# lajoiepy/cslam

Hardware: AMD Instinct MI355X
Metric: keyframes/sec (extract+match) on 100kx4096-D bank (higher is better)
Workload: dtype f32

## Files before the change

cslam_amd/csrc/wino_chain.hip:

```cpp
#include "common.h"
#include "pairs.h"
#include <hip/hip_fp16.h>

typedef float cf4 __attribute__((ext_vector_type(4)));
typedef unsigned cu2 __attribute__((ext_vector_type(2)));
typedef unsigned cu4 __attribute__((ext_vector_type(4)));

__device__ __forceinline__ void wc_at4(const cf4 m0, const cf4 m1, const cf4 m2, const cf4 m3, const cf4 m4, const cf4 m5,
                                       cf4 &s0, cf4 &s1, cf4 &s2, cf4 &s3) {
    const cf4 a = m1 + m2, bq = m1 - m2, c = m3 + m4, e = m3 - m4;
    s0 = m0 + a + c;
    s1 = bq + 2.0f * e;
    s2 = a + 4.0f * c;
    s3 = bq + 8.0f * e + m5;
}
__device__ __forceinline__ void wc_bt4(cf4 &d0, cf4 &d1, cf4 &d2, cf4 &d3, cf4 &d4, cf4 &d5) {
    const cf4 r0 = 4.0f * d0 - 5.0f * d2 + d4;
    const cf4 r1 = -4.0f * (d1 + d2) + d3 + d4;
    const cf4 r2 = 4.0f * (d1 - d2) - d3 + d4;
    const cf4 r3 = 2.0f * (d3 - d1) - d2 + d4;
    const cf4 r4 = 2.0f * (d1 - d3) - d2 + d4;
    const cf4 r5 = 4.0f * d1 - 5.0f * d3 + d5;
    d0 = r0; d1 = r1; d2 = r2; d3 = r3; d4 = r4; d5 = r5;
}

#define WC_THREADS 128
#define WC_RING 9

struct WcArgs {
    const float *mb;
    __half *vb;
    unsigned moff, voff;
    float *rp;
    int64_t mplane, vplane, mrow, vrow;
    int H, TH, Wr, tj;
    float inv, sc;
    cf4 bv;
    cf4 clim;
    bool odd;
};

template <int CG, bool OUT, bool LOAD, bool IN>
__device__ __forceinline__ void wc_step(const WcArgs &a, const int r, cf4 (&m)[36], float &vmax) {
    if (OUT) {
        cf4 s[4][6];
#pragma unroll
        for (int j = 0; j < 6; ++j)
            wc_at4(m[j], m[6 + j], m[12 + j], m[18 + j], m[24 + j], m[30 + j], s[0][j], s[1][j], s[2][j], s[3][j]);
#pragma unroll
        for (int i = 0; i < 4; ++i) {
            cf4 o[4];
            wc_at4(s[i][0], s[i][1], s[i][2], s[i][3], s[i][4], s[i][5], o[0], o[1], o[2], o[3]);
            const int h = 4 * r + i;
            float *row = a.rp + ((h % WC_RING) * a.Wr + 4 * a.tj) * CG;
            const cf4 lim = h < a.H ? a.clim : (cf4)(0.0f);
#pragma unroll
            for (int j = 0; j < 4; ++j) {
                cf4 v = __builtin_elementwise_max(o[j] * a.inv + a.bv, (cf4)(0.0f));
                v = __builtin_elementwise_min(v, (cf4)(lim[j]));
                vmax = fmaxf(fmaxf(vmax, fmaxf(v.x, v.y)), fmaxf(v.z, v.w));
                *(cf4 *)(row + j * CG) = v;
            }
        }
    }
    __syncthreads();
    if (LOAD) {
        const float *p = a.mb + (r + 1) * a.mrow;
#pragma unroll
        for (int q = 0; q < 36; ++q) m[q] = __builtin_nontemporal_load((const cf4 *)(p + q * a.mplane + a.moff));
    }
    if (IN) {
        const int h0 = 4 * (r - 1) - 1, w0 = 4 * a.tj - 1;
        const int Hr = 4 * a.TH;
        cf4 d[6][6];
#pragma unroll
        for (int i = 0; i < 6; ++i) {
            const int hh = h0 + i;
            const float *row = a.rp + ((hh + WC_RING) % WC_RING) * a.Wr * CG;
#pragma unroll
            for (int j = 0; j < 6; ++j) {
                const int ww = w0 + j;
                const bool in = (hh >= 0) & (hh < Hr) & (ww >= 0) & (ww < a.Wr);
                cf4 v = *(const cf4 *)(row + (j == 0 ? max(ww, 0) : j == 5 ? min(ww, a.Wr - 1) : ww) * CG);
                asm("" : "+v"(v));
                d[i][j] = in ? v * a.sc : (cf4)(0.0f);
            }
        }
#pragma unroll
        for (int j = 0; j < 6; ++j) wc_bt4(d[0][j], d[1][j], d[2][j], d[3][j], d[4][j], d[5][j]);
#pragma unroll
        for (int i = 0; i < 6; ++i) wc_bt4(d[i][0], d[i][1], d[i][2], d[i][3], d[i][4], d[i][5]);
        __half *o = a.vb + (r - 1) * a.vrow;
#pragma unroll
        for (int i = 0; i < 6; ++i)
#pragma unroll
            for (int j = 0; j < 6; ++j) {
                const cf4 v = d[i][j];
                const __half2 h0v = __floats2half2_rn(v.x, v.y), h1v = __floats2half2_rn(v.z, v.w);
                const __half2 l0v = __floats2half2_rn(sub_half<0>(v.x, h0v), sub_half<1>(v.y, h0v));
                const __half2 l1v = __floats2half2_rn(sub_half<0>(v.z, h1v), sub_half<1>(v.w, h1v));
                cu2 hi, lo;
                hi.x = *(const unsigned *)&h0v; hi.y = *(const unsigned *)&h1v;
                lo.x = *(const unsigned *)&l0v; lo.y = *(const unsigned *)&l1v;
                const cu2 give = a.odd ? hi : lo;
                cu2 got;
                got.x = (unsigned)__builtin_amdgcn_mov_dpp((int)give.x, 0xB1, 0xF, 0xF, true);
                got.y = (unsigned)__builtin_amdgcn_mov_dpp((int)give.y, 0xB1, 0xF, 0xF, true);
                cu4 v16;
                if (a.odd) { v16.x = got.x; v16.y = got.y; v16.z = lo.x; v16.w = lo.y; }
                else { v16.x = hi.x; v16.y = hi.y; v16.z = got.x; v16.w = got.y; }
                __builtin_nontemporal_store(v16, (cu4 *)(o + (6 * i + j) * a.vplane + a.voff));
            }
    }
    __syncthreads();
}

template <int CG>
__global__ __launch_bounds__(WC_THREADS) void wino4_chain_h2_kernel(const float *__restrict__ M, const float *__restrict__ bias,
                                                                     int B, int H, int W, int C,
                                                                     const unsigned *__restrict__ vscale, float inv_su,
                                                                     const unsigned *__restrict__ amax_x, float wl1, float bmax,
                                                                     unsigned *__restrict__ amax_out,
                                                                     unsigned *__restrict__ bound_out, __half *__restrict__ V2) {
    extern __shared__ __attribute__((aligned(16))) float ring[];
    __shared__ unsigned wg_amax;
    constexpr int C4G = CG / 4;
    WcArgs a;
    a.H = H;
    a.TH = (H + 3) >> 2;
    const int TW = (W + 3) >> 2;
    a.Wr = 4 * TW;
    const int ncg = C / CG;
    const int b = blockIdx.x / ncg, cg = blockIdx.x - b * ncg;
    a.tj = threadIdx.x / C4G;
    const int c4 = threadIdx.x % C4G;
    const int c = cg * CG + 4 * c4;
    const int64_t T = (int64_t)B * a.TH * TW;
    const int64_t t0 = (int64_t)b * a.TH * TW;
    if (threadIdx.x == 0) wg_amax = 0u;

    a.inv = inv_su / scale_le_327_68(__uint_as_float(*vscale));
    const float bound = fmaf(__uint_as_float(*amax_x), wl1, bmax);
    a.sc = scale_le_327_68(bound);
    if (blockIdx.x == 0 && threadIdx.x == 0) *bound_out = __float_as_uint(bound);
    a.bv = bias ? *(const cf4 *)(bias + c) : (cf4)(0.0f);
#pragma unroll
    for (int j = 0; j < 4; ++j) a.clim[j] = 4 * a.tj + j < W ? __builtin_inff() : 0.0f;
    a.odd = threadIdx.x & 1;
    a.mplane = T * C;
    a.vplane = T * 2 * C;
    a.mrow = (int64_t)TW * C;
    a.vrow = (int64_t)TW * 2 * C;
    a.mb = M + t0 * C + cg * CG;
    a.vb = V2 + t0 * 2 * C + cg * 2 * CG;
    a.moff = a.tj * C + 4 * c4;
    a.voff = a.tj * 2 * C + (c4 >> 3) * 64 + (4 * c4 & 31) + (a.odd ? 32 - 4 : 0);
    a.rp = ring + 4 * c4;
    float vmax = 0.0f;

    cf4 m[36];
#pragma unroll
    for (int q = 0; q < 36; ++q) m[q] = __builtin_nontemporal_load((const cf4 *)(a.mb + q * a.mplane + a.moff));
    const int TH = a.TH;
    if (TH == 1) {
        wc_step<CG, true, false, false>(a, 0, m, vmax);
    } else {
        wc_step<CG, true, true, false>(a, 0, m, vmax);
#pragma unroll 1
        for (int r = 1; r < TH - 1; ++r) wc_step<CG, true, true, true>(a, r, m, vmax);
        wc_step<CG, true, false, true>(a, TH - 1, m, vmax);
    }
    wc_step<CG, false, false, true>(a, TH, m, vmax);
#pragma unroll
    for (int o = 32; o > 0; o >>= 1) vmax = fmaxf(vmax, __shfl_xor(vmax, o, 64));
    if ((threadIdx.x & 63) == 0) atomicMax(&wg_amax, __float_as_uint(vmax));
    __syncthreads();
    if (threadIdx.x == 0 && wg_amax > *(volatile unsigned *)amax_out) atomicMax(amax_out, wg_amax);
}

template <int CG>
static int wino4_chain_launch(const float *d_M, const float *d_bias, int B, int H, int W, int C, const unsigned *d_vscale,
                              float inv_su, const unsigned *d_amax_x, float wl1, float bmax, unsigned *d_amax_out,
                              unsigned *d_bound_out, void *d_V2, void *stream) {
    const size_t lds = (size_t)WC_RING * 4 * ((W + 3) / 4) * CG * sizeof(float);
    ARG_CHECK(lds <= 144 * 1024, "map too wide for the LDS ring");
    static DeviceOnce once;
    int dev;
    if (once.todo(&dev)) {
        HIP_TRY(hipFuncSetAttribute((const void *)wino4_chain_h2_kernel<CG>, hipFuncAttributeMaxDynamicSharedMemorySize, 144 * 1024));
        once.done(dev);
    }
    hipLaunchKernelGGL(wino4_chain_h2_kernel<CG>, dim3((unsigned)((int64_t)B * (C / CG))), dim3(((W + 3) / 4) * (CG / 4)), lds, (hipStream_t)stream,
                       d_M, d_bias, B, H, W, C, d_vscale, inv_su, d_amax_x, wl1, bmax, d_amax_out, d_bound_out, (__half *)d_V2);
    HIP_TRY(hipGetLastError());
    return CSLAM_OK;
}

CSLAM_API int cslam_wino4_chain_h2_dev(const float *d_M, const float *d_bias, int B, int H, int W, int C,
                                       const unsigned *d_vscale, float inv_su, const unsigned *d_amax_x, float wl1, float bmax,
                                       unsigned *d_amax_out, unsigned *d_bound_out, void *d_V2, void *stream) {
    PTR_DEVICE(d_M);
    ARG_CHECK(d_M && d_V2 && d_vscale && d_amax_x && d_amax_out && d_bound_out, "NULL argument");
    ARG_CHECK(B >= 1 && H >= 1 && W >= 1, "empty map");
    ARG_CHECK(C >= 32 && (C % 32) == 0, "C must be a multiple of 32");
    ARG_CHECK(inv_su > 0.0f && wl1 >= 0.0f && bmax >= 0.0f, "inv_su must be positive, wl1 and bmax non-negative");
    const int TW = (W + 3) / 4;
    ARG_CHECK(TW <= 16, "maps wider than 64 pixels stay on the separate transforms");
    ARG_CHECK((int64_t)B * (C / 32) < (1LL << 31), "too many frames for one launch");
    if (TW <= 4 && (C % 128) == 0)
        return wino4_chain_launch<128>(d_M, d_bias, B, H, W, C, d_vscale, inv_su, d_amax_x, wl1, bmax, d_amax_out, d_bound_out, d_V2, stream);
    if (TW <= 8 && (C % 64) == 0)
        return wino4_chain_launch<64>(d_M, d_bias, B, H, W, C, d_vscale, inv_su, d_amax_x, wl1, bmax, d_amax_out, d_bound_out, d_V2, stream);
    return wino4_chain_launch<32>(d_M, d_bias, B, H, W, C, d_vscale, inv_su, d_amax_x, wl1, bmax, d_amax_out, d_bound_out, d_V2, stream);
}
```

Before: 19040.

## Pad LDS ring with zero halo and prescale on write to drop bounds checks

The LDS ring now has a one-pixel zero-padded border per row (Wp = 4*TW+1) and is zero-initialised, so the input-transform reads no longer need per-element bounds tests, clamping, or multiplication by the scale. The scale factor moves to the output-transform write side, and the final empty step writes zeros instead of skipping the write. The B^T transform is rewritten with explicit FMAs under contract(off) to keep rounding deterministic. Ablation variants selected by an env var are added, but only when built with CSLAM_ABLATIONS; the cost is a little more LDS and an initial zero-fill.

```diff
diff --git a/cslam_amd/csrc/wino_chain.hip b/cslam_amd/csrc/wino_chain.hip
--- a/cslam_amd/csrc/wino_chain.hip
+++ b/cslam_amd/csrc/wino_chain.hip
@@ -14,13 +14,22 @@
     s2 = a + 4.0f * c;
     s3 = bq + 8.0f * e + m5;
 }
+template <bool FUSED>
+__device__ __forceinline__ cf4 wc_4a5b(const cf4 a, const cf4 b) {
+#pragma clang fp contract(off)
+    if (FUSED) return __builtin_elementwise_fma((cf4)(-5.0f), b, 4.0f * a);
+    const cf4 t = 5.0f * b;
+    return __builtin_elementwise_fma((cf4)(4.0f), a, -t);
+}
+template <bool DOWN>
 __device__ __forceinline__ void wc_bt4(cf4 &d0, cf4 &d1, cf4 &d2, cf4 &d3, cf4 &d4, cf4 &d5) {
-    const cf4 r0 = 4.0f * d0 - 5.0f * d2 + d4;
-    const cf4 r1 = -4.0f * (d1 + d2) + d3 + d4;
-    const cf4 r2 = 4.0f * (d1 - d2) - d3 + d4;
-    const cf4 r3 = 2.0f * (d3 - d1) - d2 + d4;
-    const cf4 r4 = 2.0f * (d1 - d3) - d2 + d4;
-    const cf4 r5 = 4.0f * d1 - 5.0f * d3 + d5;
+#pragma clang fp contract(off)
+    const cf4 r0 = wc_4a5b<DOWN>(d0, d2) + d4;
+    const cf4 r1 = __builtin_elementwise_fma((cf4)(-4.0f), d1 + d2, d3) + d4;
+    const cf4 r2 = __builtin_elementwise_fma((cf4)(4.0f), d1 - d2, -d3) + d4;
+    const cf4 r3 = __builtin_elementwise_fma((cf4)(2.0f), d3 - d1, -d2) + d4;
+    const cf4 r4 = __builtin_elementwise_fma((cf4)(2.0f), d1 - d3, -d2) + d4;
+    const cf4 r5 = wc_4a5b<false>(d1, d3) + d5;
     d0 = r0; d1 = r1; d2 = r2; d3 = r3; d4 = r4; d5 = r5;
 }
 
@@ -33,35 +42,42 @@
     unsigned moff, voff;
     float *rp;
     int64_t mplane, vplane, mrow, vrow;
-    int H, TH, Wr, tj;
+    int H, Wp;
     float inv, sc;
     cf4 bv;
     cf4 clim;
     bool odd;
 };
 
-template <int CG, bool OUT, bool LOAD, bool IN>
-__device__ __forceinline__ void wc_step(const WcArgs &a, const int r, cf4 (&m)[36], float &vmax) {
+template <int CG, bool OUT, bool LOAD, bool IN, int DBG>
+__device__ __forceinline__ void wc_step(const WcArgs &a, const int r, cf4 (&m)[36], float &vmax, unsigned &sink) {
     if (OUT) {
         cf4 s[4][6];
 #pragma unroll
-        for (int j = 0; j < 6; ++j)
-            wc_at4(m[j], m[6 + j], m[12 + j], m[18 + j], m[24 + j], m[30 + j], s[0][j], s[1][j], s[2][j], s[3][j]);
+        for (int j = 0; j < 6; ++j) {
+            if (DBG == 3) s[0][j] = s[1][j] = s[2][j] = s[3][j] = m[j] + m[6 + j] + m[12 + j] + m[18 + j] + m[24 + j] + m[30 + j];
+            else wc_at4(m[j], m[6 + j], m[12 + j], m[18 + j], m[24 + j], m[30 + j], s[0][j], s[1][j], s[2][j], s[3][j]);
+        }
 #pragma unroll
         for (int i = 0; i < 4; ++i) {
             cf4 o[4];
-            wc_at4(s[i][0], s[i][1], s[i][2], s[i][3], s[i][4], s[i][5], o[0], o[1], o[2], o[3]);
+            if (DBG == 3) { o[0] = s[i][0] + s[i][4]; o[1] = s[i][1] + s[i][5]; o[2] = s[i][2]; o[3] = s[i][3]; }
+            else wc_at4(s[i][0], s[i][1], s[i][2], s[i][3], s[i][4], s[i][5], o[0], o[1], o[2], o[3]);
             const int h = 4 * r + i;
-            float *row = a.rp + ((h % WC_RING) * a.Wr + 4 * a.tj) * CG;
+            float *row = a.rp + ((h % WC_RING) * a.Wp + 1) * CG;
             const cf4 lim = h < a.H ? a.clim : (cf4)(0.0f);
 #pragma unroll
             for (int j = 0; j < 4; ++j) {
                 cf4 v = __builtin_elementwise_max(o[j] * a.inv + a.bv, (cf4)(0.0f));
                 v = __builtin_elementwise_min(v, (cf4)(lim[j]));
                 vmax = fmaxf(fmaxf(vmax, fmaxf(v.x, v.y)), fmaxf(v.z, v.w));
-                *(cf4 *)(row + j * CG) = v;
+                *(cf4 *)(row + j * CG) = v * a.sc;
             }
         }
+    } else {
+        float *row = a.rp + (((4 * r) % WC_RING) * a.Wp + 1) * CG;
+#pragma unroll
+        for (int j = 0; j < 4; ++j) *(cf4 *)(row + j * CG) = (cf4)(0.0f);
     }
     __syncthreads();
     if (LOAD) {
@@ -69,27 +85,19 @@
 #pragma unroll
         for (int q = 0; q < 36; ++q) m[q] = __builtin_nontemporal_load((const cf4 *)(p + q * a.mplane + a.moff));
     }
-    if (IN) {
-        const int h0 = 4 * (r - 1) - 1, w0 = 4 * a.tj - 1;
-        const int Hr = 4 * a.TH;
+    if (IN && DBG != 2) {
+        const int h0 = 4 * (r - 1) - 1;
         cf4 d[6][6];
 #pragma unroll
         for (int i = 0; i < 6; ++i) {
-            const int hh = h0 + i;
-            const float *row = a.rp + ((hh + WC_RING) % WC_RING) * a.Wr * CG;
-#pragma unroll
-            for (int j = 0; j < 6; ++j) {
-                const int ww = w0 + j;
-                const bool in = (hh >= 0) & (hh < Hr) & (ww >= 0) & (ww < a.Wr);
-                cf4 v = *(const cf4 *)(row + (j == 0 ? max(ww, 0) : j == 5 ? min(ww, a.Wr - 1) : ww) * CG);
-                asm("" : "+v"(v));
-                d[i][j] = in ? v * a.sc : (cf4)(0.0f);
-            }
+            const float *row = a.rp + ((h0 + i + WC_RING) % WC_RING) * a.Wp * CG;
+#pragma unroll
+            for (int j = 0; j < 6; ++j) d[i][j] = *(const cf4 *)(row + j * CG);
         }
 #pragma unroll
-        for (int j = 0; j < 6; ++j) wc_bt4(d[0][j], d[1][j], d[2][j], d[3][j], d[4][j], d[5][j]);
-#pragma unroll
-        for (int i = 0; i < 6; ++i) wc_bt4(d[i][0], d[i][1], d[i][2], d[i][3], d[i][4], d[i][5]);
+        for (int j = 0; j < 6; ++j) wc_bt4<true>(d[0][j], d[1][j], d[2][j], d[3][j], d[4][j], d[5][j]);
+#pragma unroll
+        for (int i = 0; i < 6; ++i) wc_bt4<false>(d[i][0], d[i][1], d[i][2], d[i][3], d[i][4], d[i][5]);
         __half *o = a.vb + (r - 1) * a.vrow;
 #pragma unroll
         for (int i = 0; i < 6; ++i)
@@ -109,13 +117,14 @@
                 cu4 v16;
                 if (a.odd) { v16.x = got.x; v16.y = got.y; v16.z = lo.x; v16.w = lo.y; }
                 else { v16.x = hi.x; v16.y = hi.y; v16.z = got.x; v16.w = got.y; }
-                __builtin_nontemporal_store(v16, (cu4 *)(o + (6 * i + j) * a.vplane + a.voff));
+                if (DBG == 1) sink ^= v16.x ^ v16.y ^ v16.z ^ v16.w;
+                else __builtin_nontemporal_store(v16, (cu4 *)(o + (6 * i + j) * a.vplane + a.voff));
             }
     }
     __syncthreads();
 }
 
-template <int CG>
+template <int CG, int DBG>
 __global__ __launch_bounds__(WC_THREADS) void wino4_chain_h2_kernel(const float *__restrict__ M, const float *__restrict__ bias,
                                                                      int B, int H, int W, int C,
                                                                      const unsigned *__restrict__ vscale, float inv_su,
@@ -127,16 +136,15 @@
     constexpr int C4G = CG / 4;
     WcArgs a;
     a.H = H;
-    a.TH = (H + 3) >> 2;
-    const int TW = (W + 3) >> 2;
-    a.Wr = 4 * TW;
+    const int TH = (H + 3) >> 2, TW = (W + 3) >> 2;
+    a.Wp = 4 * TW + 1;
     const int ncg = C / CG;
     const int b = blockIdx.x / ncg, cg = blockIdx.x - b * ncg;
-    a.tj = threadIdx.x / C4G;
+    const int tj = threadIdx.x / C4G;
     const int c4 = threadIdx.x % C4G;
     const int c = cg * CG + 4 * c4;
-    const int64_t T = (int64_t)B * a.TH * TW;
-    const int64_t t0 = (int64_t)b * a.TH * TW;
+    const int64_t T = (int64_t)B * TH * TW;
+    const int64_t t0 = (int64_t)b * TH * TW;
     if (threadIdx.x == 0) wg_amax = 0u;
 
     a.inv = inv_su / scale_le_327_68(__uint_as_float(*vscale));
@@ -145,7 +153,7 @@
     if (blockIdx.x == 0 && threadIdx.x == 0) *bound_out = __float_as_uint(bound);
     a.bv = bias ? *(const cf4 *)(bias + c) : (cf4)(0.0f);
 #pragma unroll
-    for (int j = 0; j < 4; ++j) a.clim[j] = 4 * a.tj + j < W ? __builtin_inff() : 0.0f;
+    for (int j = 0; j < 4; ++j) a.clim[j] = 4 * tj + j < W ? __builtin_inff() : 0.0f;
     a.odd = threadIdx.x & 1;
     a.mplane = T * C;
     a.vplane = T * 2 * C;
@@ -153,24 +161,32 @@
     a.vrow = (int64_t)TW * 2 * C;
     a.mb = M + t0 * C + cg * CG;
     a.vb = V2 + t0 * 2 * C + cg * 2 * CG;
-    a.moff = a.tj * C + 4 * c4;
-    a.voff = a.tj * 2 * C + (c4 >> 3) * 64 + (4 * c4 & 31) + (a.odd ? 32 - 4 : 0);
-    a.rp = ring + 4 * c4;
+    a.moff = tj * C + 4 * c4;
+    a.voff = tj * 2 * C + (c4 >> 3) * 64 + (4 * c4 & 31) + (a.odd ? 32 - 4 : 0);
+    a.rp = ring + 4 * tj * CG + 4 * c4;
     float vmax = 0.0f;
+    unsigned sink = 0u;
 
     cf4 m[36];
 #pragma unroll
     for (int q = 0; q < 36; ++q) m[q] = __builtin_nontemporal_load((const cf4 *)(a.mb + q * a.mplane + a.moff));
-    const int TH = a.TH;
+    for (int q = threadIdx.x; q < (WC_RING + 1) * C4G; q += blockDim.x)
+        *(cf4 *)(ring + (q / C4G) * a.Wp * CG + 4 * (q % C4G)) = (cf4)(0.0f);
+    {
+        float *row = a.rp + ((WC_RING - 1) * a.Wp + 1) * CG;
+#pragma unroll
+        for (int j = 0; j < 4; ++j) *(cf4 *)(row + j * CG) = (cf4)(0.0f);
+    }
     if (TH == 1) {
-        wc_step<CG, true, false, false>(a, 0, m, vmax);
+        wc_step<CG, true, false, false, DBG>(a, 0, m, vmax, sink);
     } else {
-        wc_step<CG, true, true, false>(a, 0, m, vmax);
+        wc_step<CG, true, true, false, DBG>(a, 0, m, vmax, sink);
 #pragma unroll 1
-        for (int r = 1; r < TH - 1; ++r) wc_step<CG, true, true, true>(a, r, m, vmax);
-        wc_step<CG, true, false, true>(a, TH - 1, m, vmax);
-    }
-    wc_step<CG, false, false, true>(a, TH, m, vmax);
+        for (int r = 1; r < TH - 1; ++r) wc_step<CG, true, true, true, DBG>(a, r, m, vmax, sink);
+        wc_step<CG, true, false, true, DBG>(a, TH - 1, m, vmax, sink);
+    }
+    wc_step<CG, false, false, true, DBG>(a, TH, m, vmax, sink);
+    if (DBG == 1 && sink == 0x9e3779b9u) vmax = 1.0f;
 #pragma unroll
     for (int o = 32; o > 0; o >>= 1) vmax = fmaxf(vmax, __shfl_xor(vmax, o, 64));
     if ((threadIdx.x & 63) == 0) atomicMax(&wg_amax, __float_as_uint(vmax));
@@ -182,16 +198,33 @@
 static int wino4_chain_launch(const float *d_M, const float *d_bias, int B, int H, int W, int C, const unsigned *d_vscale,
                               float inv_su, const unsigned *d_amax_x, float wl1, float bmax, unsigned *d_amax_out,
                               unsigned *d_bound_out, void *d_V2, void *stream) {
-    const size_t lds = (size_t)WC_RING * 4 * ((W + 3) / 4) * CG * sizeof(float);
+    const size_t lds = ((size_t)WC_RING * (4 * ((W + 3) / 4) + 1) + 1) * CG * sizeof(float);
     ARG_CHECK(lds <= 144 * 1024, "map too wide for the LDS ring");
     static DeviceOnce once;
     int dev;
     if (once.todo(&dev)) {
-        HIP_TRY(hipFuncSetAttribute((const void *)wino4_chain_h2_kernel<CG>, hipFuncAttributeMaxDynamicSharedMemorySize, 144 * 1024));
+        HIP_TRY(hipFuncSetAttribute((const void *)wino4_chain_h2_kernel<CG, 0>, hipFuncAttributeMaxDynamicSharedMemorySize, 144 * 1024));
+#ifdef CSLAM_ABLATIONS
+        HIP_TRY(hipFuncSetAttribute((const void *)wino4_chain_h2_kernel<CG, 1>, hipFuncAttributeMaxDynamicSharedMemorySize, 144 * 1024));
+        HIP_TRY(hipFuncSetAttribute((const void *)wino4_chain_h2_kernel<CG, 2>, hipFuncAttributeMaxDynamicSharedMemorySize, 144 * 1024));
+        HIP_TRY(hipFuncSetAttribute((const void *)wino4_chain_h2_kernel<CG, 3>, hipFuncAttributeMaxDynamicSharedMemorySize, 144 * 1024));
+#endif
         once.done(dev);
     }
-    hipLaunchKernelGGL(wino4_chain_h2_kernel<CG>, dim3((unsigned)((int64_t)B * (C / CG))), dim3(((W + 3) / 4) * (CG / 4)), lds, (hipStream_t)stream,
-                       d_M, d_bias, B, H, W, C, d_vscale, inv_su, d_amax_x, wl1, bmax, d_amax_out, d_bound_out, (__half *)d_V2);
+    const dim3 grid((unsigned)((int64_t)B * (C / CG))), block(((W + 3) / 4) * (CG / 4));
+#define WC_LAUNCH(D)                                                                                                                     \
+    hipLaunchKernelGGL((wino4_chain_h2_kernel<CG, D>), grid, block, lds, (hipStream_t)stream, d_M, d_bias, B, H, W, C, d_vscale, inv_su, \
+                       d_amax_x, wl1, bmax, d_amax_out, d_bound_out, (__half *)d_V2)
+#ifdef CSLAM_ABLATIONS
+    const char *e = getenv("CSLAM_WCHAIN_DBG");
+    const int dbg = e ? atoi(e) : 0;
+    if (dbg == 1) WC_LAUNCH(1);
+    else if (dbg == 2) WC_LAUNCH(2);
+    else if (dbg == 3) WC_LAUNCH(3);
+    else
+#endif
+        WC_LAUNCH(0);
+#undef WC_LAUNCH
     HIP_TRY(hipGetLastError());
     return CSLAM_OK;
 }
```

After: 19170 (median of 6 runs). No clear change (+0.7%).
